# Blaizzy/mlx-audio

Measured on AMD Instinct MI355X. Metric: audio samples/sec + real-time factor, Kokoro-82M TTS, higher is better.
Workload: dtype bf16 weights x fp32 activations: vocoder convs = fp16 hi pass (v_mfma_f32_32x32x16_f16) + block-scaled FP4 (e2m1) lo pass (v_mfma_scale_f32_32x32x64_f8f6f4 cbsz / blgp 4, OCP MX: E8M0 scale per row x 32 channels / per output column), fp32 accumulate; front end bf16 hi+lo split; 1 GPU; Kokoro-82M bf16 TTS, tokens->waveform, canonical short sentence T=80 F=264 (6.6 s @ 24 kHz); utterances_per_gpu=64, global_batch=64, samples_per_utterance=158400, parallelism=utterance-dp1, precision_mode=6, wire=fp32

## Files before the change

### include/mi355audio.h

```cpp
#ifndef MI355AUDIO_H
#define MI355AUDIO_H

#include <stdint.h>

#ifdef __cplusplus
extern "C" {
#endif

#define MI355_OK 0
#define MI355_ERR_ARG (-1)
#define MI355_ERR_LAUNCH (-2)
#define MI355_ERR_UNSUPPORTED (-3)

const char* mi355_last_error(void);
int mi355_abi_version(void);
int mi355_device_info(int dev, char* name, int name_cap, int* cu_count, int* lds_bytes);

enum { MI355_ACT_NONE = 0, MI355_ACT_LEAKY = 1, MI355_ACT_SNAKE = 2, MI355_ACT_GELU = 3,
       MI355_ACT_ELU = 4,
       MI355_ACT_SILU = 5,
       MI355_ACT_GELU_TANH = 6,
       MI355_ACT_TANH = 7 };

typedef struct {
// ... 225 lines not shown
  const float* qkv; int64_t bstride; int32_t ld;
  int32_t heads; int32_t dh; int32_t T; const int32_t* lens; int32_t B;
  float* out; int64_t out_bstride; int32_t ldo;
} mi355_attention_args;
int mi355_attention(const mi355_attention_args* a, void* stream);

typedef struct {
  const float* table; int32_t ld_table;
  int64_t table_bstride;
  const float* pos_table; int32_t ld_pos;
  const float* add_row;
  const int32_t* idx; int32_t idx_ld;
  int32_t C; int32_t L; const int32_t* lens; int32_t B;
  float* y; int64_t y_bstride; int32_t ldy;
} mi355_gather_rows_args;
int mi355_gather_rows(const mi355_gather_rows_args* a, void* stream);

int mi355_kv_head_major16(const float* kv, int64_t kv_bstride, int32_t ld, int32_t B, int32_t T, int32_t G, int32_t H, int32_t dh, void* out, int32_t out_dtype,
                          void* stream);

int mi355_broadcast_rows(const float* v, int32_t ldv, int32_t C, float* y, int64_t y_bstride, int32_t ldy,
                         int32_t L, const int32_t* lens, int32_t B, void* stream);

typedef struct {
  const float* logits; int64_t bstride; int32_t ld; int32_t bins;
  int32_t T; const int32_t* lens; int32_t B; float speed;
  const int32_t* forced_dur;
  int32_t* dur;
  float* dur_raw;
  int32_t* frames;
  int32_t* idx; int32_t idx_ld;
  int32_t max_frames;
} mi355_duration_args;
int mi355_duration_align(const mi355_duration_args* a, void* stream);

typedef struct {
  const float* x; int64_t x_bstride; int32_t ldx; int32_t C; int32_t L; const int32_t* lens; int32_t B;
  const float* pre_scale; const float* pre_shift; int32_t pre_ld;
  int32_t pre_act; float pre_slope; const float* pre_alpha;
  float* y; int64_t y_bstride; int32_t ldy;
  float* minmax;
} mi355_fake_quant_args;
int mi355_fake_quant_extrema_from_partials(const mi355_fake_quant_args* a, void* stream);
int mi355_fake_quant_u8(const mi355_fake_quant_args* a, void* stream);
int mi355_fake_quant_extrema(const mi355_fake_quant_args* a, void* stream);

typedef struct {
  const float* x; int64_t rows; int32_t ldx; int32_t D;
  const float* tables;
  const float* tables_t;
  const float* c2;
  int32_t bins; int32_t n_layers;
  int32_t* codes; int32_t ld_codes;
  float* margins;
} mi355_rvq_encode_args;
int mi355_rvq_encode(const mi355_rvq_encode_args* a, void* stream);

typedef struct {
  const float* x; int64_t x_bstride; int32_t ldx;
  const float* gate; int32_t gate_ld;
  const float* res; int64_t res_bstride; int32_t ldr;
  int32_t pre_tanh;
  float* y; int64_t y_bstride; int32_t ldy;
  int32_t B; int32_t T; int32_t C; int32_t pad;
} mi355_ecapa_rows_args;
int mi355_ecapa_rows(const mi355_ecapa_rows_args* a, void* stream);
typedef struct {
  const float* x; int64_t x_bstride; int32_t ldx;
  int32_t B; int32_t T; int32_t C;
  float eps;
  float* mean; float* std; int32_t out_ld;
} mi355_time_moments_args;
int mi355_time_moments(const mi355_time_moments_args* a, void* stream);
typedef struct {
  const float* x; int64_t x_bstride; int32_t ldx;
  const float* logits; int64_t l_bstride; int32_t ldl;
  int32_t B; int32_t T; int32_t C;
  float eps;
  float* out; int32_t out_ld;
} mi355_attentive_pool_args;
int mi355_attentive_pool(const mi355_attentive_pool_args* a, void* stream);

typedef struct {
  const float* x; int64_t x_bstride; int32_t ldx; int32_t C; int32_t L; const int32_t* lens; int32_t B;
  const float* up_filter; const float* down_filter;
  const float* alpha; const float* inv_beta;
  float* y; int64_t y_bstride; int32_t ldy;
} mi355_aa_act_args;
int mi355_aa_activation(const mi355_aa_act_args* a, void* stream);

typedef struct {
  const float* x; int64_t x_bstride; int32_t n_in; int32_t rows;
  const double* table; int32_t up; int32_t down; int32_t K; int32_t first;
  float* y; int64_t y_bstride; int32_t n_out;
} mi355_resample_args;
int mi355_resample_poly(const mi355_resample_args* a, void* stream);

typedef struct {
  const float* x; int64_t x_bstride; int32_t ldx; int32_t C; int32_t L; const int32_t* lens; int32_t B;
  const float* scale; const float* shift; int32_t pre_ld; float slope;
  const float* w;
  const float* bias;
  float* y; int64_t y_bstride; int32_t ldy;
} mi355_pool_up2_args;
int mi355_adain_pool_up2(const mi355_pool_up2_args* a, void* stream);

typedef struct {
  const float* x; int64_t x_rstride; int32_t W; int64_t rows;
  int32_t size; int32_t mode; int32_t align_corners; float scale; float half_scale;
  float* y; int64_t y_rstride;
} mi355_interp1d_args;
int mi355_interpolate1d(const mi355_interp1d_args* a, void* stream);

int mi355_conv1d_c1_k3s2(const float* x, int32_t ldx_b, int32_t Lin, const int32_t* lens_in,
                         float w0, float w1, float w2, float bias, float* y, int64_t y_bstride, int32_t ldy, int32_t col,
                         int32_t Lout, int32_t B, void* stream);

typedef struct {
  const float* f0; int32_t ld_f0; int32_t L2; const int32_t* lens2; int32_t B;
  int32_t up; int32_t H; float sr; float sine_amp; float noise_std; float voiced_thr;
  const float* rand_ini; const float* noise;
  const float* lin_w; float lin_b;
  float* phase_ws;
  float* out; int32_t ld_out;
  float* quant_ws;
  int32_t coarse_f32;
} mi355_sine_source_args;
int mi355_sine_source(const mi355_sine_source_args* a, void* stream);

typedef struct {
  const float* x; int32_t ldx; int32_t L; const int32_t* lens; int32_t B;
  int32_t n_fft; int32_t hop; const float* window;
  float* y; int64_t y_bstride; int32_t ldy;
} mi355_stft_magphase_args;
int mi355_stft_magphase(const mi355_stft_magphase_args* a, void* stream);

typedef struct {
  const float* x; int64_t x_bstride; int32_t ldx; int32_t Fr; const int32_t* lens; int32_t B;
  int32_t n_fft; int32_t hop; const float* window;
  float* audio; int32_t ld_audio;
} mi355_istft_head_args;
int mi355_istft_head(const mi355_istft_head_args* a, void* stream);

typedef struct {
  const float* x; int64_t x_bstride; int32_t ldx; int32_t Cin; int32_t L; const int32_t* lens; int32_t B;
  const uint16_t* w; const float* bias; int32_t Cout; int32_t K; int32_t dil; int32_t pad;
  int32_t pre_act; float pre_slope; int32_t precision;
  int32_t n_fft; int32_t hop; const float* window;
  float* audio; int32_t ld_audio;
} mi355_conv_post_istft_args;
int mi355_conv_post_istft(const mi355_conv_post_istft_args* a, void* stream);

typedef struct {
  const float* x; int32_t ldx; int32_t L; int32_t B;
  int32_t n_fft; int32_t hop; const float* window;
  int32_t pad_mode; int32_t n_frames;
  float* out;
} mi355_stft_args;
int mi355_stft(const mi355_stft_args* a, void* stream);

typedef struct {
  const float* x; int32_t ldx; int32_t L; int32_t B;
  int32_t n_fft; int32_t hop; const float* window; int32_t pad_mode; int32_t n_frames;
  const float* fb; int32_t n_mels; int32_t mode;
  float* out;
  float* gmax;
  float log_guard;
} mi355_logmel_args;
int mi355_logmel(const mi355_logmel_args* a, void* stream);
int mi355_logmel_finish(float* y, int64_t n_per_item, const float* gmax, int32_t B, void* stream);

typedef struct {
  const float* x; int32_t L;
  int32_t win; int32_t shift; int32_t pad; int32_t n_fft; int32_t n_frames;
  const float* window;
  const float* noise;
  float dither; float preemph;
  float* frames;
} mi355_kaldi_frames_args;
int mi355_kaldi_frames(const mi355_kaldi_frames_args* a, void* stream);
int mi355_polar_spec(const float* x, int64_t x_bstride, int32_t ldx, int32_t Fr, int32_t nb, int32_t B, float clip, float* spec, void* stream);


typedef struct {
  const float* spec; int32_t n_frames; int32_t B;
  int32_t n_fft; int32_t hop; const float* window; const float* norm;
  int32_t norm_mode;
  int32_t clamp; int32_t trim; int32_t out_len;
  float* frames_ws;
  float* out; int32_t ld_out;
} mi355_istft_args;
int mi355_istft(const mi355_istft_args* a, void* stream);

enum { MI355_KV_F32 = 0, MI355_KV_BF16 = 1, MI355_KV_F16 = 2 };
typedef struct {
  const float* q; int64_t q_bstride; int32_t ldq;
  const float* k; int64_t k_bstride; int32_t ldk;
  const float* v; int64_t v_bstride; int32_t ldv;
  int32_t heads; int32_t kv_heads; int32_t dh;
  int32_t Tq; int32_t Tk;
  const int32_t* lens_q;
  const int32_t* lens_k;
  int32_t causal; int32_t window; float scale;
  int32_t B;
  int32_t mode;
  float* out; int64_t out_bstride; int32_t ldo;
  const int32_t* k_start;
  float* split_ws; int32_t* split_cnt; int32_t nsplit;
  int64_t k_hstride; int64_t v_hstride;
  int32_t kv_dtype;
  const float* new_k; const float* new_v; int64_t new_bstride;
  const float* q_norm_w; const float* k_norm_w; float norm_eps;
  const float* rope_cos; const float* rope_sin; int32_t rope_rows; int32_t rope_mode; int32_t rope_pos;
  int32_t in_kgroups; int64_t in_kg_stride; const float* q_bias; const float* k_bias; const float* v_bias;
  const float* q_wscale; const float* k_wscale; const float* v_wscale;
  uint16_t* out_planes; int32_t planes_R; int32_t planes_dtype;
} mi355_flash_attn_args;
int mi355_flash_attention(const mi355_flash_attn_args* a, void* stream);

typedef struct {
  const float* logits; int32_t ld; int32_t V; int32_t B;
  int32_t* tokens; int32_t tokens_ld; int32_t n;
  int32_t sample_begin;
  const float* suppress_mask;
  const int32_t* blank_ids; int32_t n_blank;
  int32_t timestamp_rules;
  int32_t timestamp_begin; int32_t eot; int32_t no_timestamps;
  int32_t max_initial_timestamp_index;
  const float* gumbel; float temperature;
  float* sum_logprobs;
  float* filtered;
  const int32_t* forced_next;
  float* split_ws; int32_t* split_cnt;
} mi355_whisper_step_args;
int mi355_whisper_greedy_step(const mi355_whisper_step_args* a, void* stream);
int mi355_softmax_prob_at(const float* logits, int32_t ld, int32_t V, int32_t B, int32_t token, float* out, void* stream);

typedef struct {
  const float* x; int32_t ldx; int32_t M; int32_t K;
  const uint16_t* w; int32_t ldw; int32_t wdtype; int32_t N;
  const float* bias;
  int32_t post_act; float post_slope;
  const float* colscale;
  const float* res; int32_t ldr;
  float out_scale;
  int32_t glu;
  float* y; int32_t ldy;
  int32_t norm; const float* norm_weight; const float* norm_bias; float norm_eps;
  float* y2; int32_t ldy2; int32_t split;
  const float* wscale;
  int32_t norm_two_reads;
  const float* rope_cos; const float* rope_sin; int32_t rope_dh; int32_t rope_cols;
  const int32_t* x_ids; int32_t x_id_offset;
  float* split_ws; int32_t* split_cnt;
  int32_t y2_dtype;
  int32_t w_policy;
  const void* attn_k; const void* attn_v; int32_t attn_ld; int32_t attn_Tk; int32_t attn_heads; int32_t attn_kv_heads; int32_t attn_dh;
  float attn_scale; int32_t attn_kv_dtype;
} mi355_gemv_args;
int mi355_gemv(const mi355_gemv_args* a, void* stream);
int mi355_pack_rowmajor16_host(const float* w_host, int64_t n, int32_t dtype, uint16_t* out_host);
int mi355_pack_rowmajor_fp8_host(const float* w_host, int64_t rows, int64_t cols, uint8_t* out_host, float* scale_host);

typedef struct {
  const float* x; int64_t x_bstride; int32_t ldx;
  int32_t C; int32_t L; const int32_t* lens; int32_t B;
  const float* weight;
  float eps;
  float* y; int64_t y_bstride; int32_t ldy;
} mi355_rmsnorm_args;
int mi355_rmsnorm(const mi355_rmsnorm_args* a, void* stream);

typedef struct {
  const float* x; int64_t x_bstride; int32_t ldx;
  int32_t heads; int32_t dh; int32_t L; const int32_t* lens; int32_t B;
  const float* norm_weight; float eps;
  const float* cos_table; const float* sin_table;
  const int32_t* pos; int32_t pos_ld; int32_t pos0;
  const int32_t* pos_sub;
  int32_t rope_rows;
  int32_t rope_mode;
  float* y; int64_t y_bstride; int32_t ldy;
  const float* x2; int64_t x2_bstride; int32_t ldx2; int32_t heads2; const float* norm_weight2;
  float* y2; int64_t y2_bstride; int32_t ldy2;
} mi355_head_rope_args;
int mi355_head_norm_rope(const mi355_head_rope_args* a, void* stream);

int mi355_swiglu(const float* x, int64_t ldx, float* y, int64_t ldy, int64_t rows, int32_t I, void* stream);

typedef struct {
  const float* table; int32_t ld_table;
  const int32_t* slot_offset;
  const int32_t* ids; int64_t ids_bstride; int32_t ids_ld; int32_t ids_qstride; int32_t Q;
  const float* add; int64_t add_bstride; int32_t add_ld;
  float scale;
  int32_t C; int32_t L; const int32_t* lens; int32_t B;
  float* y; int64_t y_bstride; int32_t ldy;
} mi355_embed_sum_args;
int mi355_embed_sum(const mi355_embed_sum_args* a, void* stream);

typedef struct {
  const float* x; int64_t x_bstride; int32_t ldx; int32_t Lin; const int32_t* lens_in;
  const float* w;
  const float* bias;
  int32_t C; int32_t K; int32_t pad; int32_t stride; int32_t transpose; int32_t B;
  float* y; int64_t y_bstride; int32_t ldy; int32_t Lout;
// ... 294 lines not shown
```

### mlx_audio_amd/build.py

```python
from __future__ import annotations

import hashlib
import os
import shutil
import subprocess
import sys

HERE = os.path.dirname(os.path.abspath(__file__))
CSRC = os.path.join(HERE, "csrc")
LIBDIR = os.path.join(HERE, "lib")
LIBPATH = os.path.join(LIBDIR, "libmi355audio.so")
HEADER = os.path.join(os.path.dirname(HERE), "include", "mi355audio.h")
SOURCES = ["api.cpp", "conv_gemm.hip", "conv_ws4.hip", "conv_ws4_p4.hip", "conv_ws4_p13.hip", "conv_ws4_p5.hip", "conv_ws4_p6.hip", "conv_ws4_p5_probe.hip", "conv_ws4_fq.hip", "conv_quant.hip", "norm.hip", "group_norm.hip", "s3.hip", "conformer.hip", "narrow_attn.hip", "mid_attn.hip", "align.hip", "lstm.hip", "lstm_seq.hip", "gru.hip", "dfn.hip", "bandsplit.hip", "sanm.hip", "mossformer.hip", "attention.hip", "glue.hip", "source.hip", "fft.hip", "flash_attn.hip",
           "decode_rules.hip", "gemv.hip", "gemv_mfma.hip", "gemv_mfma_fp8.hip", "gemm_rows.hip", "rows_pipe.hip", "transformer.hip", "rvq.hip", "ecapa.hip", "sampler.hip", "stack_step.cpp"]
EXTRA_FLAGS = {"source.hip": ["-ffp-contract=off"], "dfn.hip": ["-ffp-contract=off"]}
COMMON_FLAGS = ["-fno-slp-vectorize"]


def _hipcc() -> str:
    for cand in (os.environ.get("HIPCC"), shutil.which("hipcc"), "/opt/rocm/bin/hipcc"):
        if cand and os.path.exists(cand):
            return cand
    raise RuntimeError("hipcc not found (set HIPCC=/path/to/hipcc)")


def _fingerprint() -> str:
    h = hashlib.sha256()
    for name in SOURCES + sorted(n for n in os.listdir(CSRC) if n.endswith(".h")):
        with open(os.path.join(CSRC, name), "rb") as f:
            h.update(f.read())
    with open(HEADER, "rb") as f:
        h.update(f.read())
    h.update(repr(sorted(EXTRA_FLAGS.items())).encode())
    h.update(repr(COMMON_FLAGS).encode())
    return h.hexdigest()


def build(force: bool = False, verbose: bool = True) -> str:
    os.makedirs(LIBDIR, exist_ok=True)
    stamp = os.path.join(LIBDIR, "libmi355audio.stamp")
    fp = _fingerprint()
    if not force and os.path.exists(LIBPATH) and os.path.exists(stamp) and open(stamp).read().strip() == fp:
        return LIBPATH
    hipcc = _hipcc()
    objs = []
    objdir = os.path.join(LIBDIR, "obj")
    os.makedirs(objdir, exist_ok=True)
    procs = []
    for src in SOURCES:
        obj = os.path.join(objdir, src.rsplit(".", 1)[0] + ".o")
        objs.append(obj)
        cmd = [hipcc, "--offload-arch=gfx950", "-O3", "-std=c++17", "-fPIC", *COMMON_FLAGS, *EXTRA_FLAGS.get(src, []), "-x", "hip", "-c",
               os.path.join(CSRC, src), "-o", obj]
        if verbose:
            print("[build]", " ".join(cmd), flush=True)
        procs.append((src, subprocess.Popen(cmd, stdout=subprocess.PIPE, stderr=subprocess.STDOUT, text=True)))
    for src, p in procs:
        out, _ = p.communicate()
        if p.returncode != 0:
            raise RuntimeError(f"hipcc failed on {src}:\n{out}")
        if verbose and out.strip():
            print(out)
    link = [hipcc, "--offload-arch=gfx950", "-shared", "-fPIC", "-o", LIBPATH] + objs
    if verbose:
        print("[build]", " ".join(link), flush=True)
    r = subprocess.run(link, stdout=subprocess.PIPE, stderr=subprocess.STDOUT, text=True)
    if r.returncode != 0:
        raise RuntimeError(f"link failed:\n{r.stdout}")
    with open(stamp, "w") as f:
        f.write(fp)
    return LIBPATH


if __name__ == "__main__":
    print(build(force="--force" in sys.argv))
```

### mlx_audio_amd/ops.py

```python
from __future__ import annotations

import ctypes
import math
import os
from dataclasses import dataclass
from typing import Optional, Tuple

import numpy as np
import torch

from . import _lib

ACT_NONE, ACT_LEAKY, ACT_SNAKE, ACT_GELU, ACT_ELU, ACT_SILU, ACT_GELU_TANH, ACT_TANH = 0, 1, 2, 3, 4, 5, 6, 7

PROFILE = None


def _stream() -> int:
    return torch.cuda.current_stream().cuda_stream


def profile_finalize(entries):
    torch.cuda.synchronize()
    out = []
# ... 1436 lines not shown
    kw = dict(logits=_ptr(logits), ld=logits.stride(0), V=V or logits.shape[1], B=B, suppress_mask=_ptr(suppress_mask),
              repetition_penalty=repetition_penalty, temperature=temperature, top_k=top_k, top_p=top_p, min_p=min_p, gumbel=_ptr(gumbel),
              done=_ptr(done), done_token=done_token, out=_ptr(out), out_ld=out_ld, filtered=_ptr(filtered))
    if history is not None:
        assert history.dtype == torch.int32 and history.dim() == 2 and history.stride(1) == 1
        kw.update(history=_ptr(history), hist_ld=history.stride(0), n_hist=n_hist, hist_len=_ptr(hist_len))
    if gumbel is not None:
        assert gumbel.stride(0) == logits.stride(0)
    if filtered is not None:
        assert filtered.stride(0) == logits.stride(0)
    _lib.call_struct("mi355_sample", "mi355_sample_args", _stream(), **kw)
    return out


def gather_rows(table: torch.Tensor, idx: torch.Tensor, y: torch.Tensor, *, per_batch: bool = False, pos_table=None,
                add_row=None, lens=None):
    B, L, C, ybs, ldy = _nlc(y)
    assert idx.dtype == torch.int32 and idx.dim() == 2 and idx.stride(1) == 1
    if per_batch:
        assert table.dim() == 3 and table.stride(2) == 1
        tbs, ldt = table.stride(0), table.stride(1)
    else:
        assert table.dim() == 2 and table.stride(1) == 1
        tbs, ldt = 0, table.stride(0)
    _lib.call_struct("mi355_gather_rows", "mi355_gather_rows_args", _stream(), table=_ptr(table), ld_table=ldt,
                     table_bstride=tbs, pos_table=_ptr(pos_table), ld_pos=0 if pos_table is None else pos_table.stride(0),
                     add_row=_ptr(add_row), idx=_ptr(idx), idx_ld=idx.stride(0), C=C, L=L, lens=_ptr(lens), B=B, y=_ptr(y),
                     y_bstride=ybs, ldy=ldy)
    return y


def broadcast_rows(v: torch.Tensor, y: torch.Tensor, lens=None):
    B, L, C, ybs, ldy = _nlc(y)
    assert v.dim() == 2 and v.stride(1) == 1
    lib = _lib.load()
    rc = lib.mi355_broadcast_rows(_ptr(v), v.stride(0), C, _ptr(y), ybs, ldy, L, _ptr(lens), B, _stream())
    _lib.check(rc, "mi355_broadcast_rows")
    return y


def duration_align(logits: Optional[torch.Tensor], T: int, B: int, speed: float, idx_cap: int, device, lens=None,
                   forced: Optional[torch.Tensor] = None, bins: int = 50, max_frames: int = 0):
    dur = torch.empty((B, T), dtype=torch.int32, device=device)
    raw = torch.zeros((B, T), dtype=torch.float32, device=device)
    frames = torch.empty((B,), dtype=torch.int32, device=device)
    idx = torch.zeros((B, idx_cap), dtype=torch.int32, device=device)
    kw = dict(T=T, lens=_ptr(lens), B=B, speed=speed, forced_dur=_ptr(forced), dur=_ptr(dur), dur_raw=_ptr(raw),
              frames=_ptr(frames), idx=_ptr(idx), idx_ld=idx_cap, bins=bins, max_frames=max_frames)
    if logits is not None:
        _, _, _, bs, ld = _nlc(logits)
        kw.update(logits=_ptr(logits), bstride=bs, ld=ld)
    _lib.call_struct("mi355_duration_align", "mi355_duration_args", _stream(), **kw)
    return dur, raw, frames, idx


def adain_pool_up2(x: torch.Tensor, scale, shift, slope: float, w: torch.Tensor, bias: torch.Tensor, y: torch.Tensor, lens=None):
    B, L, C, xbs, ldx = _nlc(x)
    _, _, _, ybs, ldy = _nlc(y)
    _lib.call_struct("mi355_adain_pool_up2", "mi355_pool_up2_args", _stream(), x=_ptr(x), x_bstride=xbs, ldx=ldx, C=C, L=L,
                     lens=_ptr(lens), B=B, scale=_ptr(scale), shift=_ptr(shift), pre_ld=scale.stride(0), slope=slope,
                     w=_ptr(w), bias=_ptr(bias), y=_ptr(y), y_bstride=ybs, ldy=ldy)
    return y


def aa_activation(x: torch.Tensor, y: torch.Tensor, up_filter: torch.Tensor, down_filter: torch.Tensor, alpha: torch.Tensor, inv_beta: torch.Tensor, lens=None):
    B, L, C, xbs, ldx = _nlc(x)
    _, _, _, ybs, ldy = _nlc(y)
    assert up_filter.numel() == 12 and down_filter.numel() == 12 and alpha.numel() >= C and inv_beta.numel() >= C
    _lib.call_struct("mi355_aa_activation", "mi355_aa_act_args", _stream(), x=_ptr(x), x_bstride=xbs, ldx=ldx, C=C, L=L, lens=_ptr(lens), B=B,
                     up_filter=_ptr(up_filter), down_filter=_ptr(down_filter), alpha=_ptr(alpha), inv_beta=_ptr(inv_beta), y=_ptr(y), y_bstride=ybs, ldy=ldy)
    return y


def resample_poly(x: torch.Tensor, table: torch.Tensor, up: int, down: int, first: int, n_out: int, y: Optional[torch.Tensor] = None) -> torch.Tensor:
    assert x.dim() == 2 and x.dtype == torch.float32 and x.stride(1) == 1 and table.dtype == torch.float64 and table.is_contiguous() and table.shape[1] == up
    rows, n_in = x.shape
    if y is None:
        y = torch.empty(rows, n_out, device=x.device, dtype=torch.float32)
    assert y.shape == (rows, n_out) and y.stride(1) == 1 and y.dtype == torch.float32
    _lib.call_struct("mi355_resample_poly", "mi355_resample_args", _stream(), x=_ptr(x), x_bstride=x.stride(0), n_in=n_in, rows=rows, table=_ptr(table),
                     up=up, down=down, K=table.shape[0], first=first, y=_ptr(y), y_bstride=y.stride(0), n_out=n_out)
    return y


def conv1d_c1_k3s2(x: torch.Tensor, w3, bias: float, y: torch.Tensor, col: int, lens_in=None):
    assert x.dim() == 2 and x.stride(1) == 1
    B, Lout, _, ybs, ldy = _nlc(y)
    lib = _lib.load()
    rc = lib.mi355_conv1d_c1_k3s2(_ptr(x), x.stride(0), x.shape[1], _ptr(lens_in), float(w3[0]), float(w3[1]), float(w3[2]),
                                  float(bias), _ptr(y), ybs, ldy, col, Lout, B, _stream())
    _lib.check(rc, "mi355_conv1d_c1_k3s2")
    return y


def sine_source(f0: torch.Tensor, rand_ini: torch.Tensor, noise: torch.Tensor, lin_w: torch.Tensor, lin_b: float, up: int,
                lens2=None, sr: float = 24000.0, sine_amp: float = 0.1, noise_std: float = 0.003, voiced_thr: float = 10.0, quant: bool = False,
                coarse_f32: bool = False):
    B, L2 = f0.shape
    H = rand_ini.shape[1]
    assert f0.stride(1) == 1 and noise.is_contiguous() and tuple(noise.shape) == (B, L2 * up, H)
    ws = torch.empty((B, H, L2 + 1), dtype=torch.float32, device=f0.device)
    out = torch.zeros((B, L2 * up), dtype=torch.float32, device=f0.device)
    _lib.call_struct("mi355_sine_source", "mi355_sine_source_args", _stream(), f0=_ptr(f0), ld_f0=f0.stride(0), L2=L2,
                     lens2=_ptr(lens2), B=B, up=up, H=H, sr=sr, sine_amp=sine_amp, noise_std=noise_std, voiced_thr=voiced_thr,
                     rand_ini=_ptr(rand_ini), noise=_ptr(noise), lin_w=_ptr(lin_w), lin_b=lin_b, phase_ws=_ptr(ws),
                     out=_ptr(out), ld_out=out.stride(0),
                     quant_ws=_ptr(torch.empty((B, 2), dtype=torch.float32, device=f0.device)) if quant else None, coarse_f32=int(bool(coarse_f32)))
    return out


def stft_magphase(x: torch.Tensor, n_fft: int, hop: int, window: torch.Tensor, y: torch.Tensor, lens=None):
    assert x.dim() == 2 and x.stride(1) == 1
    B, _, _, ybs, ldy = _nlc(y)
    _lib.call_struct("mi355_stft_magphase", "mi355_stft_magphase_args", _stream(), x=_ptr(x), ldx=x.stride(0), L=x.shape[1],
                     lens=_ptr(lens), B=B, n_fft=n_fft, hop=hop, window=_ptr(window), y=_ptr(y), y_bstride=ybs, ldy=ldy)
    return y


def istft_head(x: torch.Tensor, n_fft: int, hop: int, window: torch.Tensor, audio: torch.Tensor, lens=None):
    B, Fr, _, xbs, ldx = _nlc(x)
    _lib.call_struct("mi355_istft_head", "mi355_istft_head_args", _stream(), x=_ptr(x), x_bstride=xbs, ldx=ldx, Fr=Fr,
                     lens=_ptr(lens), B=B, n_fft=n_fft, hop=hop, window=_ptr(window), audio=_ptr(audio),
                     ld_audio=audio.stride(0))
    return audio


def conv_post_istft_eligible(pc: PackedConv, n_fft: int, hop: int, *, dil: int = 1, pad: int = 3, pre_act: int = ACT_LEAKY, precision: int = 2,
                             pre_fq=None) -> bool:
    return (pc.cin % 32 == 0 and pc.k == 7 and dil == 1 and pad == 3 and n_fft == 20 and hop == 5 and pc.cout == n_fft + 2 and pc.cout <= 32
            and pre_act == ACT_LEAKY and precision == 2 and not pc.f16 and not pc.mx and pre_fq is None)


def conv_post_istft(x: torch.Tensor, pc: PackedConv, n_fft: int, hop: int, window: torch.Tensor, audio: torch.Tensor, *, lens=None,
                    dil: int = 1, pad: int = 3, pre_act: int = ACT_LEAKY, pre_slope: float = 0.01, precision: int = 2, pre_fq=None):
    B, L, _, xbs, ldx = _nlc(x)
    if conv_post_istft_eligible(pc, n_fft, hop, dil=dil, pad=pad, pre_act=pre_act, precision=precision, pre_fq=pre_fq):
        assert audio.dim() == 2 and audio.stride(1) == 1 and audio.dtype == torch.float32 and audio.shape[1] >= (L - 1) * hop
        if PROFILE is not None:
            e0, e1 = torch.cuda.Event(enable_timing=True), torch.cuda.Event(enable_timing=True)
            e0.record()
            PROFILE.append(((L * B) if lens is None else lens.sum(), pc.cin, pc.cout, pc.k, dil, 0, e0, e1))
        _lib.call_struct("mi355_conv_post_istft", "mi355_conv_post_istft_args", _stream(), x=_ptr(x), x_bstride=xbs, ldx=ldx, Cin=pc.cin, L=L,
                         lens=_ptr(lens), B=B, w=_ptr(pc.w), bias=_ptr(pc.bias), Cout=pc.cout, K=pc.k, dil=dil, pad=pad, pre_act=pre_act,
                         pre_slope=pre_slope, precision=precision, n_fft=n_fft, hop=hop, window=_ptr(window), audio=_ptr(audio),
                         ld_audio=audio.stride(0))
        if PROFILE is not None:
            e1.record()
        return audio
    post = torch.empty((B, L, round_up(pc.cout, 4)), dtype=torch.float32, device=x.device)[:, :, :pc.cout]
    conv_gemm(x, pc, post, dil=dil, pad=pad, lens_in=lens, lens_out=lens, pre_act=pre_act, pre_slope=pre_slope, precision=precision, pre_fq=pre_fq)
    return istft_head(post, n_fft, hop, window, audio, lens=lens)


def stft_frames(x: torch.Tensor, n_fft: int, hop: int, window: torch.Tensor, pad_mode: int, n_frames: int):
    assert x.dim() == 2 and x.stride(1) == 1 and x.dtype == torch.float32
    B, L = x.shape
    out = torch.empty((B, n_frames, n_fft // 2 + 1, 2), dtype=torch.float32, device=x.device)
    _lib.call_struct("mi355_stft", "mi355_stft_args", _stream(), x=_ptr(x), ldx=x.stride(0), L=L, B=B, n_fft=n_fft, hop=hop,
                     window=_ptr(window), pad_mode=pad_mode, n_frames=n_frames, out=_ptr(out))
    return torch.view_as_complex(out)


def logmel(x: torch.Tensor, n_fft: int, hop: int, window: torch.Tensor, pad_mode: int, n_frames: int, fb: torch.Tensor,
           mode: int, log_guard: float = 0.0, fixed_max: Optional[float] = None):
    assert x.dim() == 2 and x.stride(1) == 1 and fb.is_contiguous()
    B, L = x.shape
    n_mels = fb.shape[0]
    out = torch.empty((B, n_frames, n_mels), dtype=torch.float32, device=x.device)
    gmax = torch.empty((B,), dtype=torch.float32, device=x.device) if mode == 0 else None
    _lib.call_struct("mi355_logmel", "mi355_logmel_args", _stream(), x=_ptr(x), ldx=x.stride(0), L=L, B=B, n_fft=n_fft,
                     hop=hop, window=_ptr(window), pad_mode=pad_mode, n_frames=n_frames, fb=_ptr(fb), n_mels=n_mels,
                     mode=mode, out=_ptr(out), gmax=None if fixed_max is not None else _ptr(gmax), log_guard=float(log_guard))
    if mode == 0:
        if fixed_max is not None:
            gmax.fill_(float(fixed_max))
        lib = _lib.load()
        rc = lib.mi355_logmel_finish(_ptr(out), n_frames * n_mels, _ptr(gmax), B, _stream())
        _lib.check(rc, "mi355_logmel_finish")
    return out


def kaldi_frames(x: torch.Tensor, win: int, shift: int, pad: int, n_fft: int, n_frames: int, window: torch.Tensor, preemph: float,
                 noise: Optional[torch.Tensor] = None, dither: float = 0.0) -> torch.Tensor:
    assert x.dim() == 1 and x.is_contiguous() and x.dtype == torch.float32 and window.numel() == win
    out = torch.empty((n_frames, n_fft), dtype=torch.float32, device=x.device)
    if noise is not None:
        assert noise.is_contiguous() and tuple(noise.shape) == (n_frames, win)
    _lib.call_struct("mi355_kaldi_frames", "mi355_kaldi_frames_args", _stream(), x=_ptr(x), L=x.numel(), win=win, shift=shift, pad=pad, n_fft=n_fft,
                     n_frames=n_frames, window=_ptr(window), noise=_ptr(noise), dither=dither, preemph=preemph, frames=_ptr(out))
    return out


def polar_spec(x: torch.Tensor, nb: int, clip: float = 1e2) -> torch.Tensor:
    B, Fr, C, xbs, ldx = _nlc(x)
    assert C >= 2 * nb
    spec = torch.empty((B, Fr, nb), dtype=torch.complex64, device=x.device)
    lib = _lib.load()
    rc = lib.mi355_polar_spec(_ptr(x), xbs, ldx, Fr, nb, B, float(clip), _ptr(torch.view_as_real(spec)), _stream())
    _lib.check(rc, "mi355_polar_spec")
    return spec


def istft_frames(spec: torch.Tensor, n_fft: int, hop: int, window: torch.Tensor, norm: torch.Tensor, norm_mode: int,
                 clamp: bool, trim: int, out_len: int):
    sr = torch.view_as_real(spec.contiguous())
    B, n_frames = spec.shape[0], spec.shape[1]
    ws = torch.empty((B, (n_frames + 1) // 2 * 2, n_fft), dtype=torch.float32, device=spec.device)
    out = torch.empty((B, out_len), dtype=torch.float32, device=spec.device)
    _lib.call_struct("mi355_istft", "mi355_istft_args", _stream(), spec=_ptr(sr), n_frames=n_frames, B=B, n_fft=n_fft,
                     hop=hop, window=_ptr(window), norm=_ptr(norm), norm_mode=norm_mode, clamp=int(clamp), trim=trim,
                     out_len=out_len, frames_ws=_ptr(ws), out=_ptr(out), ld_out=out.stride(0))
    return out
```

### mlx_audio_amd/tts/models/kokoro/engine.py

```python
from __future__ import annotations

import math
import os
from dataclasses import dataclass, field
from typing import Dict, List, Optional, Sequence

import numpy as np
import torch

from .... import ops
from ....ops import ACT_GELU, ACT_GELU_TANH, ACT_LEAKY, ACT_NONE, ACT_SNAKE, PackedConv, round_up


def fold_weight_norm(v: torch.Tensor, g: torch.Tensor, param_dtype: torch.dtype) -> torch.Tensor:
    v_ = v.to(param_dtype)
    g_ = g.to(param_dtype)
    axes = tuple(range(1, v_.dim()))
    nrm = torch.sqrt((v_ * v_).sum(dim=axes, keepdim=True))
    w = (v_ / (nrm + torch.tensor(1e-7, dtype=param_dtype))) * g_
    return w.to(torch.float32)


@dataclass
class _AdaIN:
# ... 530 lines not shown
                                                       forced=forced, bins=bins, max_frames=self.max_frames)
        frames_h = frames.cpu()
        Fs = [int(v) for v in frames_h]
        return KokoroFront(ids=[ids[b, : Ts[b]] for b in range(B)], ref_s=ref_s, d=[d[b, : Ts[b]] for b in range(B)],
                           dur=[dur[b, : Ts[b]] for b in range(B)], frames=Fs, speed=float(speed),
                           trace=dict(dur_raw=dur_raw, bert=h) if keep_trace else None,
                           padded=dict(ids=ids, lens_t=lens_t, d=d, dur=dur, frames=frames, idx=idx, gb_dec=gb_dec, gb_pred=gb_pred))

    def back(self, st: "KokoroFront", rand_ini: Optional[torch.Tensor] = None, noise: Optional[torch.Tensor] = None, noise_seed: int = 1234,
             return_intermediates: bool = False, overrides: Optional[Dict[str, torch.Tensor]] = None):
        dev, hid, sty = self.dev, self.hid, self.sty
        B = len(st.ids)
        Ts = [int(t.numel()) for t in st.ids]
        Tm = max(Ts)
        ragged = B > 1
        if st.padded is not None:
            pd = st.padded
            ids, lens_t, d, dur, frames, idx, gb_dec, gb_pred = (pd[k] for k in ("ids", "lens_t", "d", "dur", "frames", "idx", "gb_dec", "gb_pred"))
        else:
            ids = torch.nn.utils.rnn.pad_sequence([t.to(device=dev, dtype=torch.int32) for t in st.ids], batch_first=True)
            lens_t = torch.tensor(Ts, dtype=torch.int32, device=dev) if ragged else None
            ref_s = st.ref_s.to(device=dev, dtype=torch.float32).contiguous()
            s_dec = ref_s[:, :sty].contiguous()
            s_pred = ref_s[:, sty:].contiguous()
            gb_dec = self._style_proj(s_dec, self.style_dec, self.q_style_dec)
            gb_pred = self._style_proj(s_pred, self.style_pred, self.q_style_pred)
            d = torch.nn.utils.rnn.pad_sequence([t.to(dev) for t in st.d], batch_first=True).contiguous()
            forced = torch.nn.utils.rnn.pad_sequence([t.to(device=dev, dtype=torch.int32) for t in st.dur], batch_first=True).contiguous()
            cap = max(100, max((int(f) for f in st.frames), default=0) // max(Tm, 1) + 1)
            dur, _, frames, idx = ops.duration_align(None, Tm, B, st.speed, Tm * cap, dev, lens=lens_t, forced=forced)
        Fs = list(st.frames)
        dur_raw = st.trace["dur_raw"] if st.trace else None
        h = st.trace["bert"] if st.trace else None
        Fm = max(Fs)
        if Fm <= 0:
            return [self._new(1, zero=True) for _ in range(B)], [dur[b, : Ts[b]] for b in range(B)]
        idx = idx[:, :Fm]
        lens_f = frames if ragged else None
        lens_2f = frames * 2 if ragged else None

        x0 = self._new(B, Tm, hid)
        ops.gather_rows(self.te_emb, ids, x0, lens=lens_t)
        x1 = self._new(B, Tm, hid)
        for i, (pc, lw, lb) in enumerate(self.te_cnn):
            self._convq(f"text_encoder.cnn.{i}.0", x0, pc, x1, pad=(self.te_k - 1) // 2, lens_in=lens_t, lens_out=lens_t)
            ops.layernorm(x1, x0, weight=lw, bias=lb, eps=1e-5, lens=lens_t, post_act=ACT_LEAKY, post_slope=0.2)
        t_en = self._new(B, Tm, hid, zero=True)
        self._bilstm(self.te_lstm, x0, t_en, lens_t)

        en = self._new(B, Fm, hid + sty)
        ops.gather_rows(d, idx, en, per_batch=True, lens=lens_f)
        c_in = hid + 2
        dec_in = self._new(B, Fm, round_up(c_in, 32), zero=True)
        ops.gather_rows(t_en, idx, dec_in[:, :, :hid], per_batch=True, lens=lens_f)
        asr = dec_in[:, :, :hid]

        xs = self._new(B, Fm, hid, zero=True)
        self._bilstm(self.shared, en, xs, lens_f)
        curves = []
        for blocks, proj, proj_n in ((self.f0_blocks, self.f0_proj, "predictor.F0_proj"), (self.n_blocks, self.n_proj, "predictor.N_proj")):
            y0 = self._new(B, Fm, blocks[0].dout)
            self._resblk1d_fwd(blocks[0], xs, gb_pred, y0, lens_f)
            y1 = self._new(B, 2 * Fm, blocks[1].dout)
            self._resblk1d_fwd(blocks[1], y0, gb_pred, y1, lens_f, lens_2f)
            y2 = self._new(B, 2 * Fm, blocks[2].dout)
            self._resblk1d_fwd(blocks[2], y1, gb_pred, y2, lens_2f)
            curve = self._new(B, 2 * Fm, 1, zero=True)
            self._convq(proj_n, y2, proj, curve, lens_in=lens_2f, lens_out=lens_2f)
            curves.append(curve[:, :, 0])
        f0_curve, n_curve = curves
        overrides = overrides or {}
        if "f0" in overrides:
            f0_curve = overrides["f0"].to(device=dev, dtype=torch.float32).contiguous()
            assert tuple(f0_curve.shape) == (B, 2 * Fm)
        if "n" in overrides:
            n_curve = overrides["n"].to(device=dev, dtype=torch.float32).contiguous()
            assert tuple(n_curve.shape) == (B, 2 * Fm)

        f0_in, n_in = f0_curve, n_curve
        if self.qmods and self._isq("decoder.F0_conv"):
            f0_in = ops.fake_quant_u8(f0_curve[:, :, None], y=torch.zeros_like(f0_curve)[:, :, None], lens=lens_2f)[:, :, 0]
        if self.qmods and self._isq("decoder.N_conv"):
            n_in = ops.fake_quant_u8(n_curve[:, :, None], y=torch.zeros_like(n_curve)[:, :, None], lens=lens_2f)[:, :, 0]
        ops.conv1d_c1_k3s2(f0_in, self.f0_conv[0], self.f0_conv[1], dec_in, hid, lens_in=lens_2f)
        ops.conv1d_c1_k3s2(n_in, self.n_conv[0], self.n_conv[1], dec_in, hid + 1, lens_in=lens_2f)
        cd, gd, ad = self.cdim, self.gdim, self.adim
        c_cat = cd + ad + 2
        ca = self._new(B, Fm, round_up(c_cat, 32), zero=True)
        cb = self._new(B, Fm, round_up(c_cat, 32), zero=True)
        trace = {}
        self._resblk1d_fwd(self.enc_blk, dec_in[:, :, :c_in], gb_dec, ca[:, :, :cd], lens_f)
        if return_intermediates:
            trace.update(dec_in=dec_in[:, :, :c_in].clone(), enc=ca[:, :, :cd].clone())
        self._convq("decoder.asr_res.0", asr, self.asr_res, ca[:, :, cd:cd + ad], lens_in=lens_f, lens_out=lens_f, flatten=True)
        ca[:, :, cd + ad:c_cat].copy_(dec_in[:, :, hid:hid + 2])
        cb[:, :, cd:c_cat].copy_(ca[:, :, cd:c_cat])
        cur, nxt = ca, cb
        for i in range(3):
            self._resblk1d_fwd(self.dec_blks[i], cur[:, :, :c_cat], gb_dec, nxt[:, :, :cd], lens_f)
            cur, nxt = nxt, cur
            if return_intermediates:
                trace[f"dec{i}"] = cur[:, :, :cd].clone()
        xg = self._new(B, 2 * Fm, gd)
        self._resblk1d_fwd(self.dec_blks[3], cur[:, :, :c_cat], gb_dec, xg, lens_f, lens_2f)

        up = self.total_up
        L2 = 2 * Fm
        if rand_ini is None or noise is None:
            gen = torch.Generator(device=dev).manual_seed(noise_seed)
            rand_ini = torch.rand((B, 9), generator=gen, device=dev, dtype=torch.float32)
            noise = torch.randn((B, L2 * up, 9), generator=gen, device=dev, dtype=torch.float32)
        rand_ini = rand_ini.to(dev).contiguous()
        noise = noise.to(dev).contiguous()
        g_n = "decoder.generator"
        har_src = ops.sine_source(f0_curve, rand_ini, noise, self.src_w, self.src_b, up, lens2=lens_2f,
                                  quant=bool(self.qmods) and self._isq(f"{g_n}.m_source.l_linear"), coarse_f32=self.coarse_f32)
        nb2 = self.n_fft + 2
        nbp = ops.round_up(nb2, 4)
        n_har = L2 * up // self.hop + 1
        har = self._new(B, n_har, nbp, zero=True)[:, :, :nb2]
        lens_samples = frames * (2 * up) if ragged else None
        ops.stft_magphase(har_src, self.n_fft, self.hop, self.window, har, lens=lens_samples)
        if "har" in overrides:
            har.copy_(overrides["har"].to(device=dev, dtype=torch.float32))
        lens_har = lens_samples // self.hop + 1 if ragged else None
        x = xg
        L = L2
        lens_x = lens_2f
        nk = len(self.rk)
        for i, (u, k) in enumerate(zip(self.rates, self.kers)):
            last = i + 1 == len(self.rates)
            cout = self.ups[i].cout // u
            Lo = L * u + (1 if last else 0)
            lens_o = (lens_x * u + (1 if last else 0)) if ragged else None
            xsrc = self._new(B, Lo, cout)
            har_i = har
            if self.qmods and self._isq(f"{g_n}.noise_convs.{i}"):
                har_i = ops.fake_quant_u8(har, y=self._new(B, n_har, nbp, zero=True)[:, :, :nb2], lens=lens_har)
            if not last:
                sf = int(np.prod(self.rates[i + 1:]))
                self._conv(har_i, self.noise_convs[i], xsrc, lens_in=lens_har, lens_out=lens_o,
                           flat=dict(ldx=sf * nbp, x_off=-((sf + 1) // 2) * nbp, channels=nbp))
            else:
                self._conv(har_i, self.noise_convs[i], xsrc, lens_in=lens_har, lens_out=lens_o)
            if return_intermediates:
                trace[f"nconv{i}"] = xsrc.clone()
            xsrc = self._resblock1_fwd(self.noise_res[i], xsrc, gb_dec, lens_o)
            if return_intermediates:
                trace[f"nres{i}"] = xsrc.clone()
            kp = k // u
            xu = self._new(B, Lo, cout)
            lens_gemm = (lens_x + (kp - 1)) if ragged else None
            lens_ct = (lens_x * u) if ragged else None
            self._convq(f"{g_n}.ups.{i}", x, self.ups[i], xu, pad=kp - 1, lout=L + kp - 1, lens_in=lens_x, lens_out=lens_gemm, pre_act=ACT_LEAKY,
                        pre_slope=0.1, res=xsrc, up=dict(s=u, p=(k - u) // 2, cout=cout, row_off=1 if last else 0, lout=L * u, lens=lens_ct))
            if last:
                xu[:, 0, :].copy_(xsrc[:, 0, :])
            if return_intermediates:
                trace[f"xu{i}"] = xu.clone()
            acc = self._new(B, Lo, cout)
            xu_sums = torch.empty(B * cout * 2, dtype=torch.float64, device=dev)
            for j in range(nk):
                self._resblock1_fwd(self.resblocks[i * nk + j], xu, gb_dec, lens_o, out=acc, accumulate=j > 0,
                                    out_scale=(1.0 / nk) if j == nk - 1 else 1.0, x_sums=(xu_sums, j > 0))
            x, L, lens_x = acc, Lo, lens_o
            if return_intermediates:
                trace[f"stage{i}"] = acc.clone()
        audio = self._new(B, (L - 1) * self.hop, zero=True)
        post = None
        if not return_intermediates and not (self.qmods and self._isq(f"{g_n}.conv_post")):
            ops.conv_post_istft(x, self.conv_post, self.n_fft, self.hop, self.window, audio, lens=lens_x, pre_slope=0.01, precision=self._prec(self.conv_post))
        else:
            post = self._new(B, L, round_up(nb2, 4))
            self._convq(f"{g_n}.conv_post", x, self.conv_post, post[:, :, :nb2], pad=3, lens_in=lens_x, lens_out=lens_x, pre_act=ACT_LEAKY, pre_slope=0.01)
            ops.istft_head(post[:, :, :nb2], self.n_fft, self.hop, self.window, audio, lens=lens_x)
        outs = [audio[b, : Fs[b] * 2 * up] for b in range(B)]
        durs = [dur[b, : Ts[b]] for b in range(B)]
        if return_intermediates:
            return outs, durs, dict(d=d, en=en, f0=f0_curve, n=n_curve, asr=asr, t_en=t_en, dur_raw=dur_raw, har_src=har_src,
                                    har=har, bert=h, xg=xg, post=post[:, :, :nb2], dec3=xg, **trace)
        return outs, durs
```

Measured before the change: 201.5 million samples/s.

## Add dedicated polyphase upsample kernel for vocoder transposed convs

Adds a specialised HIP kernel for the Kokoro vocoder's transposed-conv upsamples (512->256 x10 and 256->128 x6). It stages leaky-ReLU'd input rows in LDS as a bf16 hi/lo split, streams weight fragments through a register ring, and runs MFMAs per phase. Bias, the residual add and the row_off copy are folded into the epilogue, replacing the generic conv_gemm up path plus a separate copy. This is meant to cut launch and memory traffic, but it applies to only two shapes and needs precision 2 with non-f16, non-MX weights; otherwise it falls back to the old path.

```diff
diff --git a/include/mi355audio.h b/include/mi355audio.h
--- a/include/mi355audio.h
+++ b/include/mi355audio.h
@@ -401,6 +401,15 @@
 int mi355_conv_post_istft(const mi355_conv_post_istft_args* a, void* stream);
 
 typedef struct {
+  const float* x; int64_t x_bstride; int32_t ldx; int32_t Cin; int32_t L; const int32_t* lens; int32_t B;
+  const uint16_t* w; const float* bias; int32_t Cout; int32_t K; int32_t u; int32_t p; int32_t row_off;
+  float slope; int32_t precision;
+  const float* res; int64_t res_bstride; int32_t ldr;
+  float* y; int64_t y_bstride; int32_t ldy;
+} mi355_upsample_polyphase_args;
+int mi355_upsample_polyphase(const mi355_upsample_polyphase_args* a, void* stream);
+
+typedef struct {
   const float* x; int32_t ldx; int32_t L; int32_t B;
   int32_t n_fft; int32_t hop; const float* window;
   int32_t pad_mode; int32_t n_frames;
diff --git a/mlx_audio_amd/build.py b/mlx_audio_amd/build.py
--- a/mlx_audio_amd/build.py
+++ b/mlx_audio_amd/build.py
@@ -11,7 +11,7 @@
 LIBDIR = os.path.join(HERE, "lib")
 LIBPATH = os.path.join(LIBDIR, "libmi355audio.so")
 HEADER = os.path.join(os.path.dirname(HERE), "include", "mi355audio.h")
-SOURCES = ["api.cpp", "conv_gemm.hip", "conv_ws4.hip", "conv_ws4_p4.hip", "conv_ws4_p13.hip", "conv_ws4_p5.hip", "conv_ws4_p6.hip", "conv_ws4_p5_probe.hip", "conv_ws4_fq.hip", "conv_quant.hip", "norm.hip", "group_norm.hip", "s3.hip", "conformer.hip", "narrow_attn.hip", "mid_attn.hip", "align.hip", "lstm.hip", "lstm_seq.hip", "gru.hip", "dfn.hip", "bandsplit.hip", "sanm.hip", "mossformer.hip", "attention.hip", "glue.hip", "source.hip", "fft.hip", "flash_attn.hip",
+SOURCES = ["api.cpp", "conv_gemm.hip", "conv_ws4.hip", "conv_ws4_p4.hip", "conv_ws4_p13.hip", "conv_ws4_p5.hip", "conv_ws4_p6.hip", "conv_ws4_p5_probe.hip", "conv_ws4_fq.hip", "upsample_poly.hip", "conv_quant.hip", "norm.hip", "group_norm.hip", "s3.hip", "conformer.hip", "narrow_attn.hip", "mid_attn.hip", "align.hip", "lstm.hip", "lstm_seq.hip", "gru.hip", "dfn.hip", "bandsplit.hip", "sanm.hip", "mossformer.hip", "attention.hip", "glue.hip", "source.hip", "fft.hip", "flash_attn.hip",
            "decode_rules.hip", "gemv.hip", "gemv_mfma.hip", "gemv_mfma_fp8.hip", "gemm_rows.hip", "rows_pipe.hip", "transformer.hip", "rvq.hip", "ecapa.hip", "sampler.hip", "stack_step.cpp"]
 EXTRA_FLAGS = {"source.hip": ["-ffp-contract=off"], "dfn.hip": ["-ffp-contract=off"]}
 COMMON_FLAGS = ["-fno-slp-vectorize"]
diff --git a/mlx_audio_amd/csrc/upsample_poly.hip b/mlx_audio_amd/csrc/upsample_poly.hip
--- /dev/null
+++ b/mlx_audio_amd/csrc/upsample_poly.hip
@@ -0,0 +1,204 @@
+#include "conv_common.h"
+
+using namespace mi355conv;
+
+namespace {
+
+constexpr int kUpThreads = 512;
+
+template <int CIN, int COUT, int U, int MF, int NF>
+__global__ __launch_bounds__(kUpThreads, 4) void upsample_poly_kernel(const mi355_upsample_polyphase_args a, const int nblk) {
+  constexpr int H = MF * 32, R = H + 1, NCH = CIN / 32;
+  constexpr int CHB = R * 64;
+  constexpr int PLANE = NCH * CHB;
+  constexpr int NFRAG = U * COUT / 32;
+  constexpr int NG = NFRAG / NF;
+  constexpr int NTp = ((U * COUT + 127) >> 7) << 2;
+  constexpr int64_t WSTEP = (int64_t)NTp * 2048;
+  constexpr int NS = NCH * 2;
+  constexpr int DEPTH = 3;
+  static_assert(NFRAG % NF == 0 && (COUT / 32) % NF == 0, "a column group lies inside one phase");
+  static_assert(H * NCH * 8 % kUpThreads == 0, "whole passes over the first H window rows");
+  extern __shared__ __attribute__((aligned(16))) char smem[];
+  char* const A_hi = smem;
+  char* const A_lo = smem + PLANE;
+
+  const int tid = threadIdx.x;
+  const int b = (int)blockIdx.x / nblk;
+  const int m0 = ((int)blockIdx.x - b * nblk) * H;
+  const int len_raw = a.lens ? a.lens[b] : a.L;
+  const int len_in = len_raw < 0 ? 0 : (len_raw > a.L ? a.L : len_raw);
+  if (m0 > len_in) return;
+  const int len_up = len_in * U;
+
+  {
+    constexpr int TOTAL = R * NCH * 8;
+    constexpr int NIT = (TOTAL + kUpThreads - 1) / kUpThreads;
+    const float* xb = a.x + (int64_t)b * a.x_bstride;
+    const float slope = a.slope;
+    float4 v[NIT];
+#pragma unroll
+    for (int i = 0; i < NIT; ++i) {
+      int idx = tid + i * kUpThreads;
+      idx = idx < TOTAL ? idx : TOTAL - 1;
+      const int c = ((idx >> 3) % NCH) * 32 + (idx & 7) * 4;
+      int gl = m0 - 1 + idx / (8 * NCH);
+      gl = gl < 0 ? 0 : (gl >= a.L ? a.L - 1 : gl);
+      v[i] = *(const float4*)(xb + (int64_t)gl * a.ldx + c);
+    }
+#pragma unroll
+    for (int i = 0; i < NIT; ++i) {
+      const int idx = tid + i * kUpThreads;
+      if (idx < TOTAL) {
+        const int c4 = (idx & 7) * 4, chunk = (idx >> 3) % NCH, r = idx / (8 * NCH);
+        const int gl = m0 - 1 + r;
+        const bool rowok = gl >= 0 && gl < len_in;
+        const float in[4] = {v[i].x, v[i].y, v[i].z, v[i].w};
+        float tt[4];
+#pragma unroll
+        for (int j = 0; j < 4; ++j) {
+          float u = in[j] + 0.0f;
+          const float m = u * slope;
+          u = u > 0.f ? u : m;
+          tt[j] = rowok ? u : 0.f;
+        }
+        uint2 ph, pl;
+        ph.x = pack_bf16x2(tt[0], tt[1]);
+        ph.y = pack_bf16x2(tt[2], tt[3]);
+        const float h0 = __builtin_bit_cast(float, ph.x << 16), h1 = __builtin_bit_cast(float, ph.x & 0xffff0000u);
+        const float h2 = __builtin_bit_cast(float, ph.y << 16), h3 = __builtin_bit_cast(float, ph.y & 0xffff0000u);
+        pl.x = pack_bf16x2(tt[0] - h0, tt[1] - h1);
+        pl.y = pack_bf16x2(tt[2] - h2, tt[3] - h3);
+        const int addr = chunk * CHB + r * 64 + ((((c4 >> 3) ^ ((r >> 2) & 3))) << 4) + ((c4 & 4) << 1);
+        *(uint2*)(A_hi + addr) = ph;
+        *(uint2*)(A_lo + addr) = pl;
+      }
+    }
+  }
+  float* const yb = a.y + (int64_t)b * a.y_bstride;
+  const float* const rb = a.res + (int64_t)b * a.res_bstride;
+  if (a.row_off && m0 == 0) {
+    for (int c = tid; c < COUT; c += kUpThreads) yb[c] = rb[c];
+  }
+  __syncthreads();
+
+  const int wave = __builtin_amdgcn_readfirstlane(tid >> 6);
+  for (int g = wave; g < NG; g += kUpThreads / 64) {
+    int lane = tid & 63;
+    asm volatile("" : "+v"(lane));
+    const int hl = lane & 31, hh = lane >> 5;
+    const int f0 = g * NF;
+    const int phase = (f0 * 32) / COUT, oc0 = f0 * 32 - phase * COUT;
+    const int nc0 = m0 * U + phase - a.p;
+    const int len_up_c = len_up > 0 ? len_up : 1;
+
+    f32x16 acc[MF][NF];
+#pragma unroll
+    for (int mf = 0; mf < MF; ++mf)
+#pragma unroll
+      for (int nf = 0; nf < NF; ++nf)
+#pragma unroll
+        for (int r = 0; r < 16; ++r) acc[mf][nf][r] = 0.f;
+
+    const char* const wfrag = (const char*)a.w + (int64_t)f0 * 2048 + lane * 16;
+    bf16x8 ring[DEPTH][2 * NF];
+    auto load_slice = [&](const int s) {
+      const char* const ws = wfrag + (int64_t)s * WSTEP;
+#pragma unroll
+      for (int f = 0; f < 2 * NF; ++f) ring[s % DEPTH][f] = *(const bf16x8*)(ws + f * 1024);
+    };
+#pragma unroll
+    for (int s = 0; s < DEPTH - 1; ++s) load_slice(s);
+
+#pragma unroll
+    for (int sl = 0; sl < NS; ++sl) {
+      if (sl + DEPTH - 1 < NS) load_slice(sl + DEPTH - 1);
+      asm volatile("" ::: "memory");
+      const int chunk = sl >> 1, tap = sl & 1;
+#pragma unroll
+      for (int kk = 0; kk < 2; ++kk) {
+        bf16x8 ah[MF], al[MF];
+#pragma unroll
+        for (int mf = 0; mf < MF; ++mf) {
+          const int row = mf * 32 + hl + tap;
+          const int addr = chunk * CHB + row * 64 + (((kk * 2 + hh) ^ ((row >> 2) & 3)) << 4);
+          ah[mf] = *(const bf16x8*)(A_hi + addr);
+          al[mf] = *(const bf16x8*)(A_lo + addr);
+        }
+#pragma unroll
+        for (int mf = 0; mf < MF; ++mf) {
+#pragma unroll
+          for (int nf = 0; nf < NF; ++nf) acc[mf][nf] = mfma16<2>(ah[mf], ring[sl % DEPTH][2 * nf + kk], acc[mf][nf]);
+#pragma unroll
+          for (int nf = 0; nf < NF; ++nf) acc[mf][nf] = mfma16<2>(al[mf], ring[sl % DEPTH][2 * nf + kk], acc[mf][nf]);
+        }
+      }
+    }
+
+    {
+      const uint32_t col = (uint32_t)(oc0 + hl) * 4u, ypb = (uint32_t)a.ldy * 4u, rpb = (uint32_t)a.ldr * 4u;
+      float bias[NF];
+#pragma unroll
+      for (int nf = 0; nf < NF; ++nf) bias[nf] = a.bias ? a.bias[oc0 + nf * 32 + hl] : 0.f;
+#pragma unroll
+      for (int mf = 0; mf < MF; ++mf) {
+        float rv[NF][16];
+#pragma unroll
+        for (int r = 0; r < 16; ++r) {
+          int nc = nc0 + (mf * 32 + (r & 3) + 8 * (r >> 2) + 4 * hh) * U;
+          nc = nc < 0 ? 0 : (nc >= len_up_c ? len_up_c - 1 : nc);
+          const uint32_t off = (uint32_t)(nc + a.row_off) * rpb + col;
+#pragma unroll
+          for (int nf = 0; nf < NF; ++nf) rv[nf][r] = *(const float*)((const char*)rb + (off + (uint32_t)(nf * 128)));
+        }
+#pragma unroll
+        for (int r = 0; r < 16; ++r) {
+          const int nc = nc0 + (mf * 32 + (r & 3) + 8 * (r >> 2) + 4 * hh) * U;
+          if (nc >= 0 && nc < len_up) {
+            const uint32_t off = (uint32_t)(nc + a.row_off) * ypb + col;
+#pragma unroll
+            for (int nf = 0; nf < NF; ++nf) *(float*)((char*)yb + (off + (uint32_t)(nf * 128))) = (acc[mf][nf][r] + bias[nf]) + rv[nf][r];
+          }
+        }
+      }
+    }
+  }
+}
+
+template <int CIN, int COUT, int U, int MF, int NF>
+int launch_up(const mi355_upsample_polyphase_args& a, hipStream_t st) {
+  constexpr int H = MF * 32;
+  constexpr int lds = 2 * (CIN / 32) * (H + 1) * 64;
+  static bool attr_set = false;
+  if (!attr_set) {
+    hipError_t e = hipFuncSetAttribute((const void*)upsample_poly_kernel<CIN, COUT, U, MF, NF>, hipFuncAttributeMaxDynamicSharedMemorySize, lds);
+    MI355_REQUIRE(e == hipSuccess, "upsample_polyphase: cannot reserve %d bytes of LDS: %s", lds, hipGetErrorString(e));
+    attr_set = true;
+  }
+  const int nblk = (a.L + 1 + H - 1) / H;
+  MI355_REQUIRE((int64_t)a.B * nblk < (int64_t)1 << 31, "upsample_polyphase: too many row blocks");
+  MI355_CLEAR_ERROR();
+  hipLaunchKernelGGL((upsample_poly_kernel<CIN, COUT, U, MF, NF>), dim3((unsigned)(a.B * nblk)), dim3(kUpThreads), lds, st, a, nblk);
+  MI355_LAUNCH_CHECK("upsample_polyphase");
+  return MI355_OK;
+}
+
+}
+
+extern "C" int mi355_upsample_polyphase(const mi355_upsample_polyphase_args* ap, void* stream) {
+  MI355_REQUIRE(ap && ap->x && ap->w && ap->res && ap->y, "upsample_polyphase: null tensor");
+  const mi355_upsample_polyphase_args a = *ap;
+  const bool s0 = a.Cin == 512 && a.Cout == 256 && a.u == 10, s1 = a.Cin == 256 && a.Cout == 128 && a.u == 6;
+  if (!(s0 || s1) || a.K != 2 * a.u || a.p != (a.K - a.u) / 2 || a.precision != 2 || (a.row_off != 0 && a.row_off != 1)) {
+    mi355_set_error("upsample_polyphase: unsupported shape (Cin=%d Cout=%d u=%d K=%d p=%d row_off=%d precision=%d)", a.Cin, a.Cout, a.u, a.K, a.p,
+                    a.row_off, a.precision);
+    return MI355_ERR_UNSUPPORTED;
+  }
+  const int64_t Lo = (int64_t)a.L * a.u + a.row_off;
+  MI355_REQUIRE(a.B > 0 && a.L > 0 && a.ldx >= a.Cin && a.ldr >= a.Cout && a.ldy >= a.Cout, "upsample_polyphase: bad shape");
+  MI355_REQUIRE(a.B == 1 || (a.x_bstride >= (int64_t)a.L * a.ldx && a.res_bstride >= Lo * a.ldr && a.y_bstride >= Lo * a.ldy), "upsample_polyphase: items overlap");
+  MI355_REQUIRE(Lo * a.ldr < ((int64_t)1 << 29) && Lo * a.ldy < ((int64_t)1 << 29), "upsample_polyphase: an item's rows exceed the 32-bit byte offsets");
+  MI355_REQUIRE((a.ldx & 3) == 0 && (a.x_bstride & 3) == 0 && (((uintptr_t)a.x | (uintptr_t)a.w) & 15) == 0, "upsample_polyphase: input rows must be 16-byte aligned");
+  if (s0) return launch_up<512, 256, 10, 1, 2>(a, (hipStream_t)stream);
+  return launch_up<256, 128, 6, 2, 1>(a, (hipStream_t)stream);
+}
diff --git a/mlx_audio_amd/ops.py b/mlx_audio_amd/ops.py
--- a/mlx_audio_amd/ops.py
+++ b/mlx_audio_amd/ops.py
@@ -1612,6 +1612,46 @@
     return istft_head(post, n_fft, hop, window, audio, lens=lens)
 
 
+UPSAMPLE_POLY_SHAPES = {(512, 256, 10): 32, (256, 128, 6): 64}
+
+
+def upsample_polyphase_eligible(pc: PackedConv, stride: int, *, pre_act: int = ACT_LEAKY, precision: int = 2, res=True, pre_fq=None) -> bool:
+    return (pc.k == 2 and stride > 0 and pc.cout % stride == 0 and (pc.cin, pc.cout // stride, stride) in UPSAMPLE_POLY_SHAPES
+            and pre_act == ACT_LEAKY and precision == 2 and not pc.f16 and not pc.mx and res is not None and pre_fq is None)
+
+
+def upsample_polyphase(x: torch.Tensor, pc: PackedConv, res: torch.Tensor, y: torch.Tensor, stride: int, *, row_off: int = 0, lens=None,
+                       pre_act: int = ACT_LEAKY, pre_slope: float = 0.1, precision: int = 2, pre_fq=None):
+    B, L, _, xbs, ldx = _nlc(x)
+    u = stride
+    cout = pc.cout // u
+    kfull = pc.k * u
+    p = (kfull - u) // 2
+    Lo = L * u + row_off
+    assert y.shape[0] == B and y.shape[1] >= Lo and y.shape[2] == cout and res.shape[0] == B and res.shape[1] >= Lo and res.shape[2] == cout
+    if upsample_polyphase_eligible(pc, u, pre_act=pre_act, precision=precision, res=res, pre_fq=pre_fq) and row_off in (0, 1):
+        _, _, _, rbs, ldr = _nlc(res)
+        _, _, _, ybs, ldy = _nlc(y)
+        assert pc.w.numel() >= _lib.load().mi355_packed_conv_weight_elems(pc.cout, pc.k, pc.cin)
+        if PROFILE is not None:
+            e0, e1 = torch.cuda.Event(enable_timing=True), torch.cuda.Event(enable_timing=True)
+            e0.record()
+            PROFILE.append((((L + 1) * B) if lens is None else (lens + 1).sum(), pc.cin, pc.cout, pc.k, 1, 1, e0, e1))
+        _lib.call_struct("mi355_upsample_polyphase", "mi355_upsample_polyphase_args", _stream(), x=_ptr(x), x_bstride=xbs, ldx=ldx, Cin=pc.cin, L=L,
+                         lens=_ptr(lens), B=B, w=_ptr(pc.w), bias=_ptr(pc.bias), Cout=cout, K=kfull, u=u, p=p, row_off=row_off, slope=pre_slope,
+                         precision=precision, res=_ptr(res), res_bstride=rbs, ldr=ldr, y=_ptr(y), y_bstride=ybs, ldy=ldy)
+        if PROFILE is not None:
+            e1.record()
+        return y
+    kp = pc.k
+    conv_gemm(x, pc, y, pad=kp - 1, lout=L + kp - 1, lens_in=lens, lens_out=None if lens is None else lens + (kp - 1), pre_act=pre_act,
+              pre_slope=pre_slope, res=res, precision=precision, pre_fq=pre_fq,
+              up=dict(s=u, p=p, cout=cout, row_off=row_off, lout=L * u, lens=None if lens is None else lens * u))
+    if row_off:
+        y[:, :row_off, :].copy_(res[:, :row_off, :])
+    return y
+
+
 def stft_frames(x: torch.Tensor, n_fft: int, hop: int, window: torch.Tensor, pad_mode: int, n_frames: int):
     assert x.dim() == 2 and x.stride(1) == 1 and x.dtype == torch.float32
     B, L = x.shape
diff --git a/mlx_audio_amd/tts/models/kokoro/engine.py b/mlx_audio_amd/tts/models/kokoro/engine.py
--- a/mlx_audio_amd/tts/models/kokoro/engine.py
+++ b/mlx_audio_amd/tts/models/kokoro/engine.py
@@ -706,10 +706,13 @@
             xu = self._new(B, Lo, cout)
             lens_gemm = (lens_x + (kp - 1)) if ragged else None
             lens_ct = (lens_x * u) if ragged else None
-            self._convq(f"{g_n}.ups.{i}", x, self.ups[i], xu, pad=kp - 1, lout=L + kp - 1, lens_in=lens_x, lens_out=lens_gemm, pre_act=ACT_LEAKY,
-                        pre_slope=0.1, res=xsrc, up=dict(s=u, p=(k - u) // 2, cout=cout, row_off=1 if last else 0, lout=L * u, lens=lens_ct))
-            if last:
-                xu[:, 0, :].copy_(xsrc[:, 0, :])
+            if not (self.qmods and self._isq(f"{g_n}.ups.{i}")) and ops.upsample_polyphase_eligible(self.ups[i], u, precision=self._prec(self.ups[i])):
+                ops.upsample_polyphase(x, self.ups[i], xsrc, xu, u, row_off=1 if last else 0, lens=lens_x, pre_slope=0.1, precision=self._prec(self.ups[i]))
+            else:
+                self._convq(f"{g_n}.ups.{i}", x, self.ups[i], xu, pad=kp - 1, lout=L + kp - 1, lens_in=lens_x, lens_out=lens_gemm, pre_act=ACT_LEAKY,
+                            pre_slope=0.1, res=xsrc, up=dict(s=u, p=(k - u) // 2, cout=cout, row_off=1 if last else 0, lout=L * u, lens=lens_ct))
+                if last:
+                    xu[:, 0, :].copy_(xsrc[:, 0, :])
             if return_intermediates:
                 trace[f"xu{i}"] = xu.clone()
             acc = self._new(B, Lo, cout)
```

Result: faster. 203.6 million samples/s, median of 6 (+1.1%).
